# andrewkwolek/dynamic-visual-slam

Hardware: AMD Instinct MI355X
Metric: frames/sec ORB+match @1280x720x2000kp (higher is better)
Workload: dtype u8

## Files before the change

dynamic-visual-slam_amd/csrc/orb.hip:

```cpp
#include <math.h>
#include <stdlib.h>
#include <string.h>
#include <algorithm>
#include <new>
#include <vector>
#include "common.h"
#include "cv_round.h"
#include "device_mem.h"
#include "io_host.h"
#ifdef DVS_TEST_HOOKS
#include "../../include/dvslam_hip_test.h"
#endif
#include "orb_kernels.h"

namespace dvs {

void launch_cand_mask(const Geom* d_geom, const Cell* d_cells, const CandMask& mk, uint32_t* cand, int* cellCount, int nimg, int c0, int c1,
                      hipStream_t st);

static inline short sat_short(int v) { return (short)(v < -32768 ? -32768 : (v > 32767 ? 32767 : v)); }
static inline uint64_t align_up(uint64_t v, uint64_t a) { return (v + a - 1) / a * a; }

}

using namespace dvs;

// ... 110 lines not shown
  hipEvent_t after_fast_event = nullptr;
  hipEvent_t gate_event = nullptr;
  bool pf_joined = false;
  const u8* next_hint = nullptr;
  struct ChainGraph { const u8* img0; uint64_t step0, fstride0; int nimg; u8* pyr; hipGraph_t graph; hipGraphExec_t exec; };
  std::vector<ChainGraph> chain_graphs;
  int env_chain_graph = -1;
  int64_t chain_graph_launches = 0;
  bool pf_valid = false;
  const u8* pf_img = nullptr; uint64_t pf_step = 0, pf_fstride = 0; int pf_nimg = 0;
  int env_cascade = -1;
  int fast_byte_dma = 0;
  int env_blur_mfma = 0;
  int env_oct_threads = 0;
  int env_host_poll = 1;
  int env_desc_order = 1;
  PinnedBuf<int> h_seq;
  DeviceBuf<int> d_ticket;
  int export_seq = 0;
  bool async_oct = false, last_async = false;
  hipStream_t tail_stream = nullptr;
  CandMask mask{};
  int last_nimg = 0;
  ImgSrc last_src{};
  StageTimer timer;
};

namespace {

void drop_chain_graphs(dvs_orb* h) {
// ... 364 lines not shown
  DVS_TRY(W.d_geom.upload(std::vector<Geom>(1, G)));
  DVS_TRY(W.d_cells.upload(tb.cells));
  DVS_TRY(W.d_tiles.upload(tb.tiles));
  DVS_TRY(W.d_strips.upload(tb.strips));
  {
    std::vector<BlurCol> bcols; std::vector<uint4> btab;
    W.blur_mfma_ok = build_blur_mfma(G, bcols, btab, W.blur_avt);
    if (W.blur_mfma_ok) { DVS_TRY(W.d_blurcols.upload(bcols)); DVS_TRY(W.d_blurtab.upload(btab)); W.n_blurcols = (int)bcols.size(); }
  }
  DVS_TRY(W.d_rgroups.upload(tb.rgroups));
  DVS_TRY(W.d_pyrtiles.upload(tb.ptiles));
  if (G.pyrLds > 0) DVS_HIP(hipFuncSetAttribute((const void*)k_pyr_cascade<256>, hipFuncAttributeMaxDynamicSharedMemorySize, 2 * G.pyrLds));
  DVS_TRY(W.d_xofs.upload(tb.xofs)); DVS_TRY(W.d_alpha.upload(tb.alpha));
  DVS_TRY(W.d_yofs.upload(tb.yofs)); DVS_TRY(W.d_beta.upload(tb.beta));
  DVS_TRY(W.ready(W.pyr.cur()));
  DVS_TRY(W.ready(W.blur.cur()));
  DVS_TRY(W.ready(W.cand.cur()));
  DVS_TRY(W.d_pts.alloc(B * G.ptsPerFrame));
  DVS_TRY(W.d_nodeof.alloc(B * G.ptsPerFrame));
  DVS_TRY(W.d_celloff.alloc(B * G.totalCells));
  DVS_TRY(W.d_candtotal.alloc(B * G.nlevels));
  for (int k = 0; k < 3; k++) DVS_TRY(W.ready(W.lvl.at(k)));
  DVS_TRY(W.d_kpsorted.alloc(B * (size_t)G.kpBlock));
  DVS_TRY(W.d_kpsortidx.alloc(B * (size_t)G.kpBlock));
  {
    std::vector<uint32_t> ident(B * (size_t)G.kpBlock);
    for (size_t f = 0; f < B; f++)
      for (int l = 0; l < G.nlevels; l++) {
        const int end = l + 1 < G.nlevels ? G.lv[l + 1].kpOff : G.kpBlock;
        for (int sl = G.lv[l].kpOff; sl < end; sl++) ident[f * G.kpBlock + sl] = (uint32_t)(sl - G.lv[l].kpOff);
      }
// ... 203 lines not shown
  hipStream_t st = h->stream;
  const bool aligned0 = (((uintptr_t)src.img0) | src.step0 | src.fstride0) % 4 == 0;
  const uint32_t allLevels = G.nlevels >= 32 ? ~0u : ((1u << G.nlevels) - 1u);
  const bool sharded = (src.levelMask & allLevels) != allLevels || src.slotted;
  const bool prefetched = h->pf_valid && h->overlap && h->pf_img == src.img0 && h->pf_step == src.step0 &&
                          h->pf_fstride == src.fstride0 && h->pf_nimg == nimg;
  h->pf_valid = false;
  bool pend = h->out_pending;
  h->out_pending = false;
  if (pend && !(prefetched && may_defer)) {
    DVS_HIP(hipStreamWaitEvent(st, h->ev_outs.cur(), 0));
    pend = false;
  }
  const bool will_defer = h->overlap && may_defer && h->output_event && h->defer_outputs && !sharded;
  const bool async = h->async_oct && prefetched && will_defer && aligned0;
  if (async) {
    DVS_TRY(W.turn(W.cand));
    if (h->tail_stream) DVS_TRY(W.turn(W.blur));
  } else if (h->last_async) {
    DVS_HIP(hipStreamWaitEvent(st, W.cand.cur().done, 0));
  }
  h->last_async = async;
  h->async_run = async ? h->async_run + 1 : 0;

  if (prefetched) {
    W.pyr.take();
    if (!h->pf_joined) DVS_HIP(hipStreamWaitEvent(st, h->ev[kEvPrefetch + h->pf_idx], 0));
  }
  h->pf_joined = false;
  src.pyr = W.pyr.cur().pyr.get();
  int topLevel = 0;
  for (int l = 0; l < G.nlevels; l++) if ((src.levelMask >> l) & 1u) topLevel = l;
  const bool want_cascade = h->env_cascade >= 0 ? h->env_cascade == 1 : nimg <= 8;
// ... 11 lines not shown
      DVS_HIP(hipEventRecord(h->ev[kEvStart], st));
      DVS_HIP(hipStreamWaitEvent(pst, h->ev[kEvStart], 0));
    }
    h->timer.begin(DVS_STAGE_PYRAMID, pst);
    DVS_TRY(launch_pyramid_chain(h, src, nimg, W.pyr.cur().pyr.get(), pst, ov, sharded ? topLevel : -1));
    h->timer.end(pst);
  }
  if (next_img0 && h->overlap && G.nlevels >= 2) DVS_TRY(launch_prefetch(h, src, nimg, next_img0, pend));

  if (h->overlap) {
    if (h->guard_event && !will_defer) { DVS_HIP(hipStreamWaitEvent(h->aux_stream, h->guard_event, 0)); h->guard_event = nullptr; }
    if (h->pf_valid && !sharded && !(h->defer_outputs && h->output_event)) { DVS_HIP(hipStreamWaitEvent(h->aux_stream, h->ev[kEvPrefetch + h->pf_idx], 0)); h->pf_joined = true; }
  }

  const bool tail = async && h->tail_stream != nullptr;
  if (tail) {
    h->timer.begin(DVS_STAGE_BLUR, st);
    launch_blur(h, src, nimg, st, cascade);
    h->timer.end(st);
  }

  if (ov) {
    int tail = G.nlevels;
    while (tail > 2 && G.lv[tail - 1].nCells * 16 < G.totalCells) tail--;
    for (int l = 0; l <= tail && l < G.nlevels; l++) {
      const int lastl = l == tail ? G.nlevels - 1 : l;
      if (lastl > 0) DVS_HIP(hipStreamWaitEvent(st, h->ev_level[lastl], 0));
      h->timer.begin(DVS_STAGE_FAST, st, l == 0);
      launch_fast(h, src, nimg, st, G.lv[l].cellBase, G.lv[lastl].cellBase + G.lv[lastl].nCells);
      h->timer.end(st);
    }
// ... 5 lines not shown
    } else {
      launch_fast(h, src, nimg, st, 0, G.totalCells);
    }
    h->timer.end(st);
  }
  hipStream_t bst = h->overlap ? h->aux_stream : st;
  hipEvent_t ev_fastdone = h->after_fast_event ? h->after_fast_event : h->ev[kEvFork];
  if (h->after_fast_event || h->overlap) DVS_HIP(hipEventRecord(ev_fastdone, st));

  if (pend) {
    DVS_TRY(W.turn(W.lvl));
  }
  hipStream_t qs = async ? bst : st;
  if (async) DVS_HIP(hipStreamWaitEvent(bst, ev_fastdone, 0));
  const int blurRows = (G.blurStrips + kOctTMax / 64 - 1) / (kOctTMax / 64);
  const bool fuse_blur = h->single_stream && !async && !sharded && !(h->env_blur_mfma && W.blur_mfma_ok) &&
                         blur_stream_ok(h, src, cascade) && (long)nimg * (G.nlevels + blurRows) <= 256;
  h->timer.begin(DVS_STAGE_OCTREE, qs);
  if (fuse_blur) {
    if (h->guard_event) { DVS_HIP(hipStreamWaitEvent(qs, h->guard_event, 0)); h->guard_event = nullptr; }
    hipLaunchKernelGGL(k_octree_blur, dim3(nimg, G.nlevels + blurRows), dim3(kOctTMax), W.octree_smem, qs, W.d_geom.get(), W.cand.cur().cand.get(), W.cand.cur().cellcount.get(),
                       W.d_celloff.get(), W.d_pts.get(), W.d_nodeof.get(), W.d_candtotal.get(), W.lvl.cur().lvlkp.get(), W.lvl.cur().lvlcount.get(), W.octree_nmax, W.octree_ptscap, src.levelMask,
                       G.nlevels, W.d_strips.get(), G.blurStrips, src, W.blur.cur().blur.get());
  } else {
    launch_octree(h, nimg, qs, src.levelMask, async && G.nlevels * nimg > 256);
  }
  h->timer.end(qs);
  if (async) { DVS_HIP(hipEventRecord(W.cand.cur().done, qs)); W.cand.cur().done_valid = true; }

  if (async) {}
  else if (bst != st) DVS_HIP(hipStreamWaitEvent(bst, ev_fastdone, 0));
  else if (h->guard_event) DVS_HIP(hipStreamWaitEvent(st, h->guard_event, 0));
  hipEvent_t late_guard = bst != st ? h->guard_event : nullptr;
  h->guard_event = nullptr;
  if (!tail && !fuse_blur) {
    h->timer.begin(DVS_STAGE_BLUR, bst);
    launch_blur(h, src, nimg, bst, cascade);
    h->timer.end(bst);
  }

  hipStream_t dst = st;
  if (will_defer) {
    dst = tail ? h->tail_stream : bst;
    if (tail) {
      DVS_HIP(hipStreamWaitEvent(dst, W.cand.cur().done, 0));
    } else if (!async) {
      DVS_HIP(hipEventRecord(h->ev[kEvOct], st));
      DVS_HIP(hipStreamWaitEvent(bst, h->ev[kEvOct], 0));
    }
    if (late_guard) DVS_HIP(hipStreamWaitEvent(dst, late_guard, 0));
  } else if (bst != st) {
    DVS_HIP(hipEventRecord(h->ev[kEvBlur], bst));
    DVS_HIP(hipStreamWaitEvent(st, h->ev[kEvBlur], 0));
  }
  h->timer.begin(DVS_STAGE_DESCRIBE, dst);
  if (h->env_desc_order && nimg >= 16) {
    hipLaunchKernelGGL(k_kp_order, dim3(nimg, G.nlevels), dim3(256), 0, dst, W.d_geom.get(), W.lvl.cur().lvlkp.get(), W.lvl.cur().lvlcount.get(), W.d_kpsorted.get(), W.d_kpsortidx.get());
    hipLaunchKernelGGL(k_describe, dim3((G.kpBlock + 4 * kDescKP - 1) / (4 * kDescKP), nimg), dim3(256), 0, dst, W.d_geom.get(), src, W.blur.cur().blur.get(),
                       W.d_kpsorted.get(), W.d_kpsortidx.get(), W.lvl.cur().lvlcount.get(), d_kps, d_desc, d_nout, capacity);
  } else {
    hipLaunchKernelGGL(k_describe, dim3((G.kpBlock + 4 * kDescKP - 1) / (4 * kDescKP), nimg), dim3(256), 0, dst, W.d_geom.get(), src, W.blur.cur().blur.get(),
                       W.lvl.cur().lvlkp.get(), W.d_kpident.get(), W.lvl.cur().lvlcount.get(), d_kps, d_desc, d_nout, capacity);
  }
  h->timer.end(dst);
  if (will_defer) {
    h->ev_outs.advance();
    h->out_gen++;
    DVS_HIP(hipEventRecord(h->ev_outs.cur(), dst));
    DVS_HIP(hipEventRecord(h->output_event, dst));
    h->out_pending = true;
    h->gate_event = nullptr;
  } else {
    h->gate_event = (may_defer && h->output_event) ? h->output_event : h->ev[kEvEnd];
    DVS_HIP(hipEventRecord(h->gate_event, st));
  }
  DVS_HIP(hipGetLastError());
  h->last_nimg = nimg;
  h->last_src = src;
// ... 34 lines not shown
  if (on_stream) {
    h->stream = ext;
  } else {
    const hipError_t e = h->own_stream.create();
    if (e != hipSuccess) { delete h; set_error("hipStreamCreate: %s", hipGetErrorString(e)); return DVS_ERR_HIP; }
    h->stream = h->own_stream;
  }
  h->single_stream = single_stream;
  h->overlap = env_int("DVS_NO_OVERLAP", 0) == 0 && !single_stream;
  h->env_cascade = env_int("DVS_CASCADE", -1);
  h->env_chain_graph = env_int("DVS_CHAIN_GRAPH", -1);
  h->env_blur_mfma = env_int("DVS_BLUR_MFMA", 0);
  h->env_host_poll = env_int("DVS_HOST_POLL", 1);
  h->env_oct_threads = env_int("DVS_OCT_T", 0);
  h->env_desc_order = env_int("DVS_DESC_ORDER", 1);
  if (h->env_oct_threads != 0 && h->env_oct_threads != kOctT && h->env_oct_threads != kOctTMax) h->env_oct_threads = 0;
  h->fast_byte_dma = probe_byte_dma(device, h->stream) && env_int("DVS_FAST_BYTE_DMA", 1);
  bool ok = single_stream || (h->aux_stream.create(-1) == hipSuccess && h->pf_stream.create(1) == hipSuccess);
  for (Event& e : h->ev) ok = ok && e.create() == hipSuccess;
  for (Event& e : h->ev_outs.slot) ok = ok && e.create() == hipSuccess;
  for (int l = 1; l < params->nlevels; l++) ok = ok && h->ev_level[l].create() == hipSuccess;
  h->ev_outs.rewind(h->ring - 1);
  if (!ok) {
    dvs_orb_destroy(h);
    set_error("stream / event creation failed");
    return DVS_ERR_HIP;
  }
  build_ctor_tables(h);
  *out = h;
  return DVS_OK;
// ... 263 lines not shown
                                  dvs_keypoint* kps, uint8_t* desc, int32_t capacity, int32_t* n_out) {
  DVS_ARG(h && n_out);
  *n_out = 0;
  if (!gray || rows <= 0 || cols <= 0) { set_error("empty image"); return DVS_ERR_EMPTY; }
  const uint8_t* one[1] = {gray};
  const uint8_t* onem[1] = {mask};
  return dvs_orb_extract_batch_masked(h, one, 1, rows, cols, step, mask ? onem : nullptr, mask_step, kps, desc, capacity, n_out);
}

dvs_status dvs_orb_get_level(dvs_orb* h, int32_t frame, int32_t level, int32_t blurred, uint8_t* dst, int32_t cap_bytes) {
  DVS_ARG(h && dst && h->ws.d_geom.get() && frame >= 0 && frame < h->last_nimg && level >= 0 && level < h->ws.geom.nlevels);
  const LevelGeom& L = h->ws.geom.lv[level];
  if ((int64_t)L.w * L.h > cap_bytes) return DVS_ERR_CAPACITY;
  DVS_HIP(hipSetDevice(h->device));
  DVS_HIP(hipStreamSynchronize(h->stream));
  if (level == 0 && !blurred) {
    DVS_HIP(hipMemcpy2D(dst, L.w, h->last_src.img0 + (uint64_t)frame * h->last_src.fstride0, h->last_src.step0, L.w, L.h, hipMemcpyDeviceToHost));
  } else {
    const u8* base = (blurred ? h->ws.blur.cur().blur.get() : h->ws.pyr.cur().pyr.get()) + (uint64_t)frame * h->ws.geom.frameBytes + L.off;
    DVS_HIP(hipMemcpy2D(dst, L.w, base, L.pitch, L.w, L.h, hipMemcpyDeviceToHost));
  }
  return DVS_OK;
}

static dvs_status read_packed(dvs_orb* h, const uint32_t* dsrc, int n, int32_t* xys) {
  std::vector<uint32_t> tmp(n);
  if (n) DVS_HIP(hipMemcpy(tmp.data(), dsrc, (size_t)n * 4, hipMemcpyDeviceToHost));
  for (int i = 0; i < n; i++) { xys[3 * i] = pt_x(tmp[i]); xys[3 * i + 1] = pt_y(tmp[i]); xys[3 * i + 2] = pt_s(tmp[i]); }
  return DVS_OK;
}
// ... 6 lines not shown
  DVS_HIP(hipMemcpy(&cnt, h->ws.d_candtotal.get() + frame * h->ws.geom.nlevels + level, 4, hipMemcpyDeviceToHost));
  *n = cnt;
  if (cnt > cap) return DVS_ERR_CAPACITY;
  return read_packed(h, h->ws.d_pts.get() + (uint64_t)frame * h->ws.geom.ptsPerFrame + h->ws.geom.lv[level].ptsOff, cnt, xys);
}

DVS_HOOK dvs_status dvs_orb_get_level_keypoints(dvs_orb* h, int32_t frame, int32_t level, int32_t* xys, int32_t cap, int32_t* n) {
  DVS_ARG(h && xys && n && h->ws.d_geom.get() && frame >= 0 && frame < h->last_nimg && level >= 0 && level < h->ws.geom.nlevels);
  DVS_HIP(hipSetDevice(h->device));
  DVS_HIP(hipStreamSynchronize(h->stream));
  int cnt = 0;
  DVS_HIP(hipMemcpy(&cnt, h->ws.lvl.cur().lvlcount.get() + frame * h->ws.geom.nlevels + level, 4, hipMemcpyDeviceToHost));
  *n = cnt;
  if (cnt > cap) return DVS_ERR_CAPACITY;
  return read_packed(h, h->ws.lvl.cur().lvlkp.get() + (uint64_t)frame * h->ws.geom.kpBlock + h->ws.geom.lv[level].kpOff, cnt, xys);
}

DVS_HOOK dvs_status dvs_orb_enable_stage_timing(dvs_orb* h, int32_t on) {
  DVS_ARG(h);
  h->timer.resolve();
  h->timer.on = on != 0;
  return DVS_OK;
}

DVS_HOOK dvs_status dvs_orb_get_stage_times(dvs_orb* h, double* ms, int64_t* calls, int32_t reset) {
  DVS_ARG(h);
  DVS_HIP(hipSetDevice(h->device));
  DVS_HIP(hipStreamSynchronize(h->stream));
  h->timer.resolve();
  for (int i = 0; i < DVS_STAGE_COUNT; i++) { if (ms) ms[i] = h->timer.ms[i]; if (calls) calls[i] = h->timer.calls[i]; }
// ... 62 lines not shown
```

dynamic-visual-slam_amd/csrc/orb_kernels.h:

```cpp
#pragma once
#include <hip/hip_runtime.h>
#include "glibc_sincosf.h"
#include "lsort.h"
#include "orb_geom.h"
#include "orb_device_common.h"

namespace dvs {

typedef uint8_t u8;

struct ImgSrc {
  const u8* img0;
  uint64_t step0;
  uint64_t fstride0;
  u8* pyr;
  uint32_t levelMask;
  int32_t slotted;
};

__device__ __forceinline__ const u8* level_ptr(const Geom* g, const ImgSrc& s, int f, int l, int& pitch) {
  if (l == 0) { pitch = (int)s.step0; return s.img0 + (uint64_t)f * s.fstride0; }
  pitch = g->lv[l].pitch;
  return s.pyr + (uint64_t)f * g->frameBytes + g->lv[l].off;
}
// ... 1653 lines not shown
  uint32_t* outI = sortedIdx + (uint64_t)f * g->kpBlock + L.kpOff;
  for (int i = threadIdx.x; i < n; i += 256) {
    const uint32_t pk = in[i];
    key[i] = ((uint32_t)(pt_y(pk) >> 5) << 20) | ((uint32_t)(pt_x(pk) >> 7) << 12) | (uint32_t)i;
  }
  __syncthreads();
  for (int i = threadIdx.x; i < n; i += 256) {
    const uint32_t k = key[i];
    int rank = 0;
    for (int j = 0; j < n; j++) rank += key[j] < k ? 1 : 0;
    outK[rank] = in[i];
    outI[rank] = (uint32_t)i;
  }
}

__global__ __launch_bounds__(256) void k_describe(const Geom* __restrict__ g, ImgSrc src, const u8* __restrict__ blur,
                                                  const uint32_t* __restrict__ lvlKp, const uint32_t* __restrict__ lvlKpIdx, const int* __restrict__ lvlKpCount,
                                                  dvs_keypoint* __restrict__ outKp, u8* __restrict__ outDesc,
                                                  int* __restrict__ nOut, int capacity) {
  typedef uint4 __attribute__((aligned(1))) uint4u;
  __shared__ __attribute__((aligned(16))) u8 win[4][2][kWinRows * kWinPitch];
  DVS_CHAIN_PRIO();
  const int wg = xcd_contiguous_id();
  const int f = wg / (int)gridDim.x, bx = wg - f * (int)gridDim.x;
  const int lane = lane_id();
  const int wv = __builtin_amdgcn_readfirstlane(threadIdx.x >> 6);
  const int nl = g->nlevels;
  const int* cnt = lvlKpCount + f * nl;
  const int slot0 = (bx * 4 + wv) * kDescKP;
  if (bx == 0 && threadIdx.x == 0) {
    if (src.slotted) {
      for (int l = 0; l < nl; l++) nOut[f * nl + l] = cnt[l];
    } else {
      int total = 0;
      for (int l = 0; l < nl; l++) total += cnt[l];
      nOut[f] = min(total, capacity);
// ... 22 lines not shown
  const int pitchL = lvl == 0 ? (int)src.step0 : g->lv[lvl].pitch;
  const u8* blurL = blur + pyrOff;
  const int bpL = g->lv[lvl].pitch;
#define DVS_RL(v, i) __builtin_amdgcn_readlane((int)(v), (i))
#define DVS_RLP(p, i) reinterpret_cast<const u8*>(((uint64_t)(uint32_t)DVS_RL((uint32_t)((uint64_t)(p) >> 32), i) << 32) | (uint32_t)DVS_RL((uint32_t)(uint64_t)(p), i))
  const int prow = min(lane >> 1, 2 * kHalfPatch), half = lane & 1;
  const int v = prow - kHalfPatch;
  const int pcol = half ? 1 : -kHalfPatch;
  uint4 d[kDescKP];
#pragma unroll
  for (int i = 0; i < kDescKP; i++) {
    const u8* ib = DVS_RLP(imgL, i);
    const int pi = DVS_RL(pitchL, i), xi = DVS_RL(x, i), yi = DVS_RL(y, i);
    d[i] = *reinterpret_cast<const uint4u*>(ib + (uint32_t)(mul_i24(yi + v, pi) + xi + pcol));
  }
  const int e0 = lane, e1 = 64 + lane;
  const int wr0 = e0 / 3, wc0 = e0 - 3 * wr0, wr1 = min(e1 / 3, kWinRows - 1), wc1 = e1 - 3 * (e1 / 3);
  const bool w1ok = e1 < kWinRows * 3;
  static_assert(kDescKP == 8, "the window registers below are named per keypoint");
  uint4 wq0_0, wq0_1, wq0_2, wq0_3, wq0_4, wq0_5, wq0_6, wq0_7, wq1_0, wq1_1, wq1_2, wq1_3, wq1_4, wq1_5, wq1_6, wq1_7;
#define DVS_REQUEST_WINDOW(i)                                                                                  \
  {                                                                                                            \
    const u8* bb = DVS_RLP(blurL, i);                                                                          \
    const int bp = DVS_RL(bpL, i), xi = DVS_RL(x, i), yi = DVS_RL(y, i);                                       \
    const int xa = (xi - kWinR) & ~3;   \
    const u8* o = bb + (int64_t)(yi - kWinR) * bp + xa;                                                        \
    wq0_##i = *reinterpret_cast<const uint4*>(o + (uint32_t)(mul_i24(wr0, bp) + 16 * wc0));                    \
    wq1_##i = *reinterpret_cast<const uint4*>(o + (uint32_t)(mul_i24(wr1, bp) + 16 * wc1));                    \
  }
  DVS_REQUEST_WINDOW(0) DVS_REQUEST_WINDOW(1) DVS_REQUEST_WINDOW(2) DVS_REQUEST_WINDOW(3)
  float px0[4], py0[4], px1[4], py1[4];
#pragma unroll
  for (int r = 0; r < 4; r++) {
    const int pat = reinterpret_cast<const int*>(c_pattern)[64 * r + lane];
    px0[r] = (float)(int8_t)(pat & 0xff); py0[r] = (float)(int8_t)((pat >> 8) & 0xff);
    px1[r] = (float)(int8_t)((pat >> 16) & 0xff); py1[r] = (float)(int8_t)((pat >> 24) & 0xff);
  }
  const uint32_t* wt = g->icw[lane];
  const uint32_t w0 = wt[0], w1 = wt[1], w2 = wt[2], w3 = wt[3], w4 = wt[4], w5 = wt[5], w6 = wt[6], w7 = wt[7];
  int q[2 * kDescKP];
#pragma unroll
  for (int i = 0; i < kDescKP; i++) {
    uint32_t su = __builtin_amdgcn_udot4(d[i].x, w0, 0u, false);
    su = __builtin_amdgcn_udot4(d[i].y, w1, su, false);
    su = __builtin_amdgcn_udot4(d[i].z, w2, su, false);
    su = __builtin_amdgcn_udot4(d[i].w, w3, su, false);
    uint32_t sm = __builtin_amdgcn_udot4(d[i].x, w4, 0u, false);
    sm = __builtin_amdgcn_udot4(d[i].y, w5, sm, false);
    sm = __builtin_amdgcn_udot4(d[i].z, w6, sm, false);
    sm = __builtin_amdgcn_udot4(d[i].w, w7, sm, false);
    q[i] = (int)su - kHalfPatch * (int)sm;
    q[kDescKP + i] = v * (int)sm;
  }
  DVS_REQUEST_WINDOW(4) DVS_REQUEST_WINDOW(5) DVS_REQUEST_WINDOW(6) DVS_REQUEST_WINDOW(7)
#define DVS_BFLY(n, o)                                        \
  {                                                           \
    const bool hi = (lane & (o)) != 0;                        \
    _Pragma("unroll") for (int j = 0; j < (n); j++) {         \
      const int keep = hi ? q[(n) + j] : q[j];                \
      const int send = hi ? q[j] : q[(n) + j];                \
      q[j] = keep + __shfl_xor(send, (o));                    \
    }                                                         \
  }
  DVS_BFLY(8, 32) DVS_BFLY(4, 16) DVS_BFLY(2, 8) DVS_BFLY(1, 4)
#undef DVS_BFLY
  int tot = q[0];
  tot += __shfl_xor(tot, 2);
  tot += __shfl_xor(tot, 1);
  const int other = __shfl_xor(tot, 32);
// ... 28 lines not shown
      const float fr0 = rowv[0], fr1 = rowv[1], fc0 = colv[0], fc1 = colv[1];
      const int r0 = __builtin_bit_cast(int, fr0), r1 = __builtin_bit_cast(int, fr1);
      const int c0 = __builtin_bit_cast(int, fc0), c1 = __builtin_bit_cast(int, fc1);
      const int t0 = wl[mad_i24(r0, kWinPitch, c0) + bco];
      const int t1 = wl[mad_i24(r1, kWinPitch, c1) + bco];
      words[r] = __ballot(t0 < t1);
    }
    if ((vmask >> i) & 1u) {
      const int gii = DVS_RL(giL, i);
      if (lane < 4) {
        const unsigned long long w = lane == 0 ? words[0] : lane == 1 ? words[1] : lane == 2 ? words[2] : words[3];
        reinterpret_cast<unsigned long long*>(outDesc + ((uint64_t)f * capacity + gii) * 32)[lane] = w;
      }
    }
  };
  brief(0, wq0_0, wq1_0); brief(1, wq0_1, wq1_1); brief(2, wq0_2, wq1_2); brief(3, wq0_3, wq1_3);
  brief(4, wq0_4, wq1_4); brief(5, wq0_5, wq1_5); brief(6, wq0_6, wq1_6); brief(7, wq0_7, wq1_7);
  const float angle = __shfl(angleK, kCsLane * (lane & 7));
  if (lane < kDescKP && valid) {
    dvs_keypoint kp;
    kp.x = (float)x; kp.y = (float)y;
    if (level != 0) { kp.x = __fmul_rn(kp.x, L.scale); kp.y = __fmul_rn(kp.y, L.scale); }
    kp.size = L.kpSize;
    kp.angle = angle;
    kp.response = (float)pt_s(pk);
    kp.octave = level;
    kp.class_id = -1;
    outKp[(uint64_t)f * capacity + gi] = kp;
  }
#undef DVS_REQUEST_WINDOW
#undef DVS_RL
#undef DVS_RLP
// ... 56 lines not shown
```

dynamic-visual-slam_amd/csrc/util.hip:

```cpp
#include <stdlib.h>
#include <string.h>
#include "common.h"
#ifdef DVS_TEST_HOOKS
#include "../../include/dvslam_hip_test.h"
#include "block_ops.h"
#include "device_mem.h"
#endif

extern "C" char** environ;

namespace dvs {

static thread_local char g_err[1024] = "";

void set_error(const char* fmt, ...) {
  va_list ap;
  va_start(ap, fmt);
  vsnprintf(g_err, sizeof(g_err), fmt, ap);
  va_end(ap);
}

namespace {
struct EnvSwitch { const char* name; int allowed[4]; int nallowed; };
const EnvSwitch kSwitches[] = {
    {"DVS_NO_OVERLAP", {0, 1}, 2},
    {"DVS_CASCADE", {-1, 0, 1}, 3},
    {"DVS_CHAIN_GRAPH", {-1, 0, 1}, 3},
    {"DVS_BLUR_MFMA", {0, 1, 2}, 3},
    {"DVS_HOST_POLL", {0, 1}, 2},
    {"DVS_OCT_T", {0, 256, 512}, 3},
    {"DVS_DESC_ORDER", {0, 1}, 2},
    {"DVS_FAST_BYTE_DMA", {0, 1}, 2},
    {"DVS_MATCH_MFMA", {0, 1}, 2},
    {"DVS_MATCH_LDS", {0, 1}, 2},
    {"DVS_LM_POLL", {0, 1}, 2},
    {"DVS_LM_SPECULATE", {0, 1}, 2},
};
const EnvSwitch* find_switch(const char* name, size_t len) {
  for (const EnvSwitch& s : kSwitches)
    if (strlen(s.name) == len && strncmp(s.name, name, len) == 0) return &s;
  return nullptr;
}
}

dvs_status env_check() {
  for (char** e = environ; e && *e; e++) {
    if (strncmp(*e, "DVS_", 4) != 0) continue;
    const char* eq = strchr(*e, '=');
    if (!eq) continue;
    const EnvSwitch* s = find_switch(*e, (size_t)(eq - *e));
    if (!s) {
      set_error("unknown environment switch %.*s (the library reads: DVS_NO_OVERLAP DVS_CASCADE DVS_CHAIN_GRAPH DVS_BLUR_MFMA DVS_HOST_POLL DVS_OCT_T "
                "DVS_DESC_ORDER DVS_FAST_BYTE_DMA DVS_MATCH_MFMA DVS_MATCH_LDS DVS_LM_POLL DVS_LM_SPECULATE)", (int)(eq - *e), *e);
      return DVS_ERR_ARG;
    }
    char* end = nullptr;
    const long v = strtol(eq + 1, &end, 10);
    bool ok = end != eq + 1 && *end == 0;
    if (ok) { ok = false; for (int i = 0; i < s->nallowed; i++) ok = ok || s->allowed[i] == (int)v; }
    if (!ok) {
      char list[64] = ""; size_t o = 0;
      for (int i = 0; i < s->nallowed; i++) o += (size_t)snprintf(list + o, sizeof(list) - o, "%s%d", i ? ", " : "", s->allowed[i]);
      set_error("%s=%s: not a value of this switch (allowed: %s)", s->name, eq + 1, list);
      return DVS_ERR_ARG;
    }
  }
  return DVS_OK;
}
// ... 255 lines not shown
```

dynamic-visual-slam_amd/dvslam_amd/_lib.py:

```python
import ctypes as C
import os
import subprocess
import numpy as np

_PKG = os.path.dirname(os.path.dirname(os.path.abspath(__file__)))
SO_PATH = os.environ.get("DVSLAM_HIP_SO") or os.path.join(_PKG, "lib", "libdvslam_hip.so")

KP_DTYPE = np.dtype([("x", "<f4"), ("y", "<f4"), ("size", "<f4"), ("angle", "<f4"), ("response", "<f4"),
                     ("octave", "<i4"), ("class_id", "<i4")])

STATUS = {0: "DVS_OK", -1: "DVS_ERR_EMPTY", -2: "DVS_ERR_UNSUPPORTED", -3: "DVS_ERR_CAPACITY", -4: "DVS_ERR_HIP",
          -5: "DVS_ERR_NO_DEVICE", -6: "DVS_ERR_ARG"}


class DvsError(RuntimeError):
    def __init__(self, code, msg):
        super().__init__(f"{STATUS.get(code, code)}: {msg}")
        self.code = code


class OrbParams(C.Structure):
    _fields_ = [("nfeatures", C.c_int32), ("scale_factor", C.c_float), ("nlevels", C.c_int32), ("ini_th_fast", C.c_int32),
                ("min_th_fast", C.c_int32), ("gauss_kernel", C.c_int32 * 7), ("max_batch", C.c_int32)]

# ... 260 lines not shown
def _bind_hooks(L):
    vp, i32, sz, dbl = C.c_void_p, C.c_int32, C.c_size_t, C.c_double
    L.dvs_orb_use_own_stream.argtypes = [vp]
    L.dvs_orb_set_overlap.argtypes = [vp, i32]
    L.dvs_matcher_use_own_stream.argtypes = [vp]
    L.dvs_orb_hint_next_batch_device.argtypes = [vp, vp]
    L.dvs_orb_set_after_fast_event.argtypes = [vp, vp]
    L.dvs_orb_set_output_event.argtypes = [vp, vp]
    L.dvs_orb_set_defer_outputs.argtypes = [vp, i32]
    L.dvs_orb_set_reuse_guard_event.argtypes = [vp, vp]
    L.dvs_orb_set_async_quadtree.argtypes = [vp, i32]
    L.dvs_orb_set_tail_stream.argtypes = [vp, vp]
    L.dvs_orb_chain_graph_launches.argtypes = [vp]; L.dvs_orb_chain_graph_launches.restype = C.c_int64
    L.dvs_orb_get_candidates.argtypes = [vp, i32, i32, vp, i32, C.POINTER(i32)]
    L.dvs_orb_get_level_keypoints.argtypes = [vp, i32, i32, vp, i32, C.POINTER(i32)]
    L.dvs_orb_enable_stage_timing.argtypes = [vp, i32]
    L.dvs_orb_get_stage_times.argtypes = [vp, vp, vp, i32]
    L.dvs_orb_create_single_stream.argtypes = [C.POINTER(OrbParams), i32, C.POINTER(vp)]
    L.dvs_orb_create_on_stream.argtypes = [C.POINTER(OrbParams), i32, vp, C.POINTER(vp)]
    L.dvs_pipeline_extractor.argtypes = [vp]; L.dvs_pipeline_extractor.restype = vp
    L.dvs_pipeline_matcher.argtypes = [vp]; L.dvs_pipeline_matcher.restype = vp
    L.dvs_pipeline_match_stream.argtypes = [vp]; L.dvs_pipeline_match_stream.restype = vp


def lib():
    global _lib
    if _lib is not None:
        return _lib
    if not os.path.exists(SO_PATH):
        raise RuntimeError(f"{SO_PATH} not found: build it with `make -C {_PKG}` (hipcc --offload-arch=gfx950); "
# ... 147 lines not shown
```

dynamic-visual-slam_amd/dvslam_amd/orb.py:

```python
import ctypes as C
import numpy as np
from ._lib import lib, test_lib, check, ptr, OrbParams, KP_DTYPE, DvsError

STAGES = ("pyramid", "fast", "octree", "blur", "describe")


class ORBextractor:

    def __init__(self, nfeatures=1000, scaleFactor=1.2, nlevels=8, iniThFAST=20, minThFAST=7, device=0, max_batch=1,
                 gauss_kernel=None, hooks=False):
        self._L = test_lib() if hooks else lib()
        self.hooks = bool(hooks)
        p = OrbParams(nfeatures, scaleFactor, nlevels, iniThFAST, minThFAST, (C.c_int32 * 7)(*(gauss_kernel or [0] * 7)), max_batch)
        h = C.c_void_p()
        check(self._L.dvs_orb_create(C.byref(p), device, C.byref(h)))
        self._h = h
        self.nfeatures, self.nlevels, self.scaleFactor, self.device, self.max_batch = nfeatures, nlevels, scaleFactor, device, max_batch
        self.capacity = self._L.dvs_orb_max_keypoints(self._h)
        self._honour_mask = False

    @classmethod
    def from_handle(cls, handle, nfeatures, nlevels, scaleFactor, device, max_batch, L=None):
        o = cls.__new__(cls)
        o._L, o._h, o._owned = (L or lib()), C.c_void_p(handle), False
# ... 170 lines not shown

    def candidates(self, l, frame=0):
        cap = 1 << 20
        buf = np.zeros((cap, 3), np.int32)
        n = C.c_int32()
        check(self._L.dvs_orb_get_candidates(self._h, frame, l, ptr(buf), cap, C.byref(n)))
        return buf[:n.value].copy()

    def level_keypoints(self, l, frame=0):
        cap = self.nfeatures + 64
        buf = np.zeros((cap, 3), np.int32)
        n = C.c_int32()
        check(self._L.dvs_orb_get_level_keypoints(self._h, frame, l, ptr(buf), cap, C.byref(n)))
        return buf[:n.value].copy()

    def enable_stage_timing(self, on=True):
        check(self._L.dvs_orb_enable_stage_timing(self._h, int(on)))

    def stage_times(self, reset=True):
        ms = np.zeros(5, np.float64); calls = np.zeros(5, np.int64)
        check(self._L.dvs_orb_get_stage_times(self._h, ptr(ms), ptr(calls), int(reset)))
        return dict(zip(STAGES, ms.tolist())), dict(zip(STAGES, calls.tolist()))
```

Measured before the change: 149,100.

## Fuse Gaussian blur into describe kernel for large deferred batches

Adds an inline-blur variant of k_describe that blurs a small window around each keypoint in LDS using packed dot-product instructions, instead of relying on a separate full-image blur pass. For large deferred batches it skips the whole blur kernel and the write and read of the blurred pyramid. The blurred image is then produced lazily only when a debug accessor asks for it. The cost is redundant blur work where keypoint windows overlap, more register and LDS pressure in describe, and a slower border path.

```diff
diff --git a/dynamic-visual-slam_amd/csrc/orb.hip b/dynamic-visual-slam_amd/csrc/orb.hip
--- a/dynamic-visual-slam_amd/csrc/orb.hip
+++ b/dynamic-visual-slam_amd/csrc/orb.hip
@@ -10,6 +10,7 @@
 #include "io_host.h"
 #ifdef DVS_TEST_HOOKS
 #include "../../include/dvslam_hip_test.h"
+#include "../../include/dvslam_hip_test_describe.h"
 #endif
 #include "orb_kernels.h"
 
@@ -150,6 +151,8 @@
   int env_blur_mfma = 0;
   int env_oct_threads = 0;
   int env_host_poll = 1;
+  int env_desc_inline = -1;
+  bool blur_current = false;
   int env_desc_order = 1;
   PinnedBuf<int> h_seq;
   DeviceBuf<int> d_ticket;
@@ -544,7 +547,6 @@
   DVS_TRY(W.d_xofs.upload(tb.xofs)); DVS_TRY(W.d_alpha.upload(tb.alpha));
   DVS_TRY(W.d_yofs.upload(tb.yofs)); DVS_TRY(W.d_beta.upload(tb.beta));
   DVS_TRY(W.ready(W.pyr.cur()));
-  DVS_TRY(W.ready(W.blur.cur()));
   DVS_TRY(W.ready(W.cand.cur()));
   DVS_TRY(W.d_pts.alloc(B * G.ptsPerFrame));
   DVS_TRY(W.d_nodeof.alloc(B * G.ptsPerFrame));
@@ -778,9 +780,12 @@
   }
   const bool will_defer = h->overlap && may_defer && h->output_event && h->defer_outputs && !sharded;
   const bool async = h->async_oct && prefetched && will_defer && aligned0;
+  constexpr int kInlineBlurMinBatch = 64;
+  const bool inline_blur = h->env_desc_inline >= 0 ? h->env_desc_inline == 1 : (will_defer && nimg >= kInlineBlurMinBatch && !h->env_blur_mfma);
+  if (!inline_blur) DVS_TRY(W.ready(W.blur.cur()));
   if (async) {
     DVS_TRY(W.turn(W.cand));
-    if (h->tail_stream) DVS_TRY(W.turn(W.blur));
+    if (h->tail_stream && !inline_blur) DVS_TRY(W.turn(W.blur));
   } else if (h->last_async) {
     DVS_HIP(hipStreamWaitEvent(st, W.cand.cur().done, 0));
   }
@@ -822,7 +827,7 @@
   }
 
   const bool tail = async && h->tail_stream != nullptr;
-  if (tail) {
+  if (tail && !inline_blur) {
     h->timer.begin(DVS_STAGE_BLUR, st);
     launch_blur(h, src, nimg, st, cascade);
     h->timer.end(st);
@@ -858,7 +863,7 @@
   hipStream_t qs = async ? bst : st;
   if (async) DVS_HIP(hipStreamWaitEvent(bst, ev_fastdone, 0));
   const int blurRows = (G.blurStrips + kOctTMax / 64 - 1) / (kOctTMax / 64);
-  const bool fuse_blur = h->single_stream && !async && !sharded && !(h->env_blur_mfma && W.blur_mfma_ok) &&
+  const bool fuse_blur = !inline_blur && h->single_stream && !async && !sharded && !(h->env_blur_mfma && W.blur_mfma_ok) &&
                          blur_stream_ok(h, src, cascade) && (long)nimg * (G.nlevels + blurRows) <= 256;
   h->timer.begin(DVS_STAGE_OCTREE, qs);
   if (fuse_blur) {
@@ -877,7 +882,7 @@
   else if (h->guard_event) DVS_HIP(hipStreamWaitEvent(st, h->guard_event, 0));
   hipEvent_t late_guard = bst != st ? h->guard_event : nullptr;
   h->guard_event = nullptr;
-  if (!tail && !fuse_blur) {
+  if (!tail && !fuse_blur && !inline_blur) {
     h->timer.begin(DVS_STAGE_BLUR, bst);
     launch_blur(h, src, nimg, bst, cascade);
     h->timer.end(bst);
@@ -898,14 +903,17 @@
     DVS_HIP(hipStreamWaitEvent(st, h->ev[kEvBlur], 0));
   }
   h->timer.begin(DVS_STAGE_DESCRIBE, dst);
-  if (h->env_desc_order && nimg >= 16) {
+  const bool ordered = h->env_desc_order && nimg >= 16;
+  if (ordered)
     hipLaunchKernelGGL(k_kp_order, dim3(nimg, G.nlevels), dim3(256), 0, dst, W.d_geom.get(), W.lvl.cur().lvlkp.get(), W.lvl.cur().lvlcount.get(), W.d_kpsorted.get(), W.d_kpsortidx.get());
-    hipLaunchKernelGGL(k_describe, dim3((G.kpBlock + 4 * kDescKP - 1) / (4 * kDescKP), nimg), dim3(256), 0, dst, W.d_geom.get(), src, W.blur.cur().blur.get(),
-                       W.d_kpsorted.get(), W.d_kpsortidx.get(), W.lvl.cur().lvlcount.get(), d_kps, d_desc, d_nout, capacity);
-  } else {
-    hipLaunchKernelGGL(k_describe, dim3((G.kpBlock + 4 * kDescKP - 1) / (4 * kDescKP), nimg), dim3(256), 0, dst, W.d_geom.get(), src, W.blur.cur().blur.get(),
-                       W.lvl.cur().lvlkp.get(), W.d_kpident.get(), W.lvl.cur().lvlcount.get(), d_kps, d_desc, d_nout, capacity);
-  }
+  const uint32_t* kpv = ordered ? W.d_kpsorted.get() : W.lvl.cur().lvlkp.get();
+  const uint32_t* kpi = ordered ? W.d_kpsortidx.get() : W.d_kpident.get();
+  const dim3 dgrid((G.kpBlock + 4 * kDescKP - 1) / (4 * kDescKP), nimg);
+  if (inline_blur)
+    hipLaunchKernelGGL(k_describe<true>, dgrid, dim3(256), 0, dst, W.d_geom.get(), src, (const u8*)nullptr, kpv, kpi, W.lvl.cur().lvlcount.get(), d_kps, d_desc, d_nout, capacity);
+  else
+    hipLaunchKernelGGL(k_describe<false>, dgrid, dim3(256), 0, dst, W.d_geom.get(), src, (const u8*)W.blur.cur().blur.get(), kpv, kpi, W.lvl.cur().lvlcount.get(), d_kps, d_desc, d_nout, capacity);
+  h->blur_current = !inline_blur;
   h->timer.end(dst);
   if (will_defer) {
     h->ev_outs.advance();
@@ -970,6 +978,7 @@
   h->env_host_poll = env_int("DVS_HOST_POLL", 1);
   h->env_oct_threads = env_int("DVS_OCT_T", 0);
   h->env_desc_order = env_int("DVS_DESC_ORDER", 1);
+  h->env_desc_inline = env_int("DVS_DESC_INLINE_BLUR", -1);
   if (h->env_oct_threads != 0 && h->env_oct_threads != kOctT && h->env_oct_threads != kOctTMax) h->env_oct_threads = 0;
   h->fast_byte_dma = probe_byte_dma(device, h->stream) && env_int("DVS_FAST_BYTE_DMA", 1);
   bool ok = single_stream || (h->aux_stream.create(-1) == hipSuccess && h->pf_stream.create(1) == hipSuccess);
@@ -1263,6 +1272,12 @@
   if ((int64_t)L.w * L.h > cap_bytes) return DVS_ERR_CAPACITY;
   DVS_HIP(hipSetDevice(h->device));
   DVS_HIP(hipStreamSynchronize(h->stream));
+  if (blurred && !h->blur_current) {
+    DVS_TRY(h->ws.ready(h->ws.blur.cur()));
+    launch_blur(h, h->last_src, h->last_nimg, h->stream, false);
+    DVS_HIP(hipStreamSynchronize(h->stream));
+    h->blur_current = true;
+  }
   if (level == 0 && !blurred) {
     DVS_HIP(hipMemcpy2D(dst, L.w, h->last_src.img0 + (uint64_t)frame * h->last_src.fstride0, h->last_src.step0, L.w, L.h, hipMemcpyDeviceToHost));
   } else {
@@ -1299,6 +1314,51 @@
   *n = cnt;
   if (cnt > cap) return DVS_ERR_CAPACITY;
   return read_packed(h, h->ws.lvl.cur().lvlkp.get() + (uint64_t)frame * h->ws.geom.kpBlock + h->ws.geom.lv[level].kpOff, cnt, xys);
+}
+
+DVS_HOOK dvs_status dvs_orb_describe_level_keypoints(dvs_orb* h, int32_t frame, const int32_t* counts, const int32_t* xys, int32_t inline_blur,
+                                                     dvs_keypoint* kps, uint8_t* desc, int32_t cap, int32_t* n_out) {
+  DVS_ARG(h && counts && xys && kps && desc && n_out && h->ws.d_geom.get() && frame >= 0 && frame < h->last_nimg);
+  Workspace& W = h->ws;
+  const Geom& G = W.geom;
+  DVS_HIP(hipSetDevice(h->device));
+  DVS_HIP(hipStreamSynchronize(h->stream));
+  std::vector<uint32_t> lk((size_t)G.kpBlock, 0u);
+  std::vector<int> cnt((size_t)h->last_nimg * G.nlevels, 0);
+  int total = 0;
+  for (int l = 0; l < G.nlevels; l++) {
+    const LevelGeom& L = G.lv[l];
+    DVS_ARG(counts[l] >= 0 && counts[l] <= L.N + 4);
+    for (int i = 0; i < counts[l]; i++, xys += 3) {
+      DVS_ARG(xys[0] >= kEdge && xys[0] < L.w - kEdge && xys[1] >= kEdge && xys[1] < L.h - kEdge && xys[2] >= 0 && xys[2] < 256);
+      lk[(size_t)L.kpOff + i] = pack_pt(xys[0] - kMinBorder, xys[1] - kMinBorder, xys[2]);
+    }
+    cnt[(size_t)frame * G.nlevels + l] = counts[l];
+    total += counts[l];
+  }
+  DVS_ARG(total <= cap && total <= G.outCap);
+  DVS_HIP(hipMemcpy(W.lvl.cur().lvlkp.get() + (uint64_t)frame * G.kpBlock, lk.data(), lk.size() * 4, hipMemcpyHostToDevice));
+  DVS_HIP(hipMemcpy(W.lvl.cur().lvlcount.get(), cnt.data(), cnt.size() * sizeof(int), hipMemcpyHostToDevice));
+  if (!inline_blur && !h->blur_current) {
+    DVS_TRY(W.ready(W.blur.cur()));
+    launch_blur(h, h->last_src, h->last_nimg, h->stream, false);
+    h->blur_current = true;
+  }
+  ImgSrc src = h->last_src;
+  src.slotted = 0;
+  const dim3 dgrid((G.kpBlock + 4 * kDescKP - 1) / (4 * kDescKP), h->last_nimg);
+  if (inline_blur)
+    hipLaunchKernelGGL(k_describe<true>, dgrid, dim3(256), 0, h->stream, W.d_geom.get(), src, (const u8*)nullptr, (const uint32_t*)W.lvl.cur().lvlkp.get(),
+                       (const uint32_t*)W.d_kpident.get(), (const int*)W.lvl.cur().lvlcount.get(), W.d_kps.get(), W.d_desc.get(), W.d_nout.get(), G.outCap);
+  else
+    hipLaunchKernelGGL(k_describe<false>, dgrid, dim3(256), 0, h->stream, W.d_geom.get(), src, (const u8*)W.blur.cur().blur.get(), (const uint32_t*)W.lvl.cur().lvlkp.get(),
+                       (const uint32_t*)W.d_kpident.get(), (const int*)W.lvl.cur().lvlcount.get(), W.d_kps.get(), W.d_desc.get(), W.d_nout.get(), G.outCap);
+  DVS_HIP(hipGetLastError());
+  DVS_HIP(hipStreamSynchronize(h->stream));
+  *n_out = total;
+  DVS_HIP(hipMemcpy(kps, W.d_kps.get() + (uint64_t)frame * G.outCap, (size_t)total * sizeof(dvs_keypoint), hipMemcpyDeviceToHost));
+  DVS_HIP(hipMemcpy(desc, W.d_desc.get() + (uint64_t)frame * G.outCap * 32, (size_t)total * 32, hipMemcpyDeviceToHost));
+  return DVS_OK;
 }
 
 DVS_HOOK dvs_status dvs_orb_enable_stage_timing(dvs_orb* h, int32_t on) {
diff --git a/dynamic-visual-slam_amd/csrc/orb_kernels.h b/dynamic-visual-slam_amd/csrc/orb_kernels.h
--- a/dynamic-visual-slam_amd/csrc/orb_kernels.h
+++ b/dynamic-visual-slam_amd/csrc/orb_kernels.h
@@ -1691,12 +1691,20 @@
   }
 }
 
+constexpr int kIbR = kWinR + 3, kIbRows = 2 * kIbR + 1;
+constexpr int kIbGroups = 10, kIbItems = kIbRows * kIbGroups;
+constexpr int kIbIters = (kIbItems + 63) / 64;
+constexpr int kIbPitch = 8 * kIbGroups, kIbWave = kIbRows * kIbPitch;
+typedef uint32_t IbWords __attribute__((ext_vector_type(3)));
+
+template <bool kInlineBlur>
 __global__ __launch_bounds__(256) void k_describe(const Geom* __restrict__ g, ImgSrc src, const u8* __restrict__ blur,
                                                   const uint32_t* __restrict__ lvlKp, const uint32_t* __restrict__ lvlKpIdx, const int* __restrict__ lvlKpCount,
                                                   dvs_keypoint* __restrict__ outKp, u8* __restrict__ outDesc,
                                                   int* __restrict__ nOut, int capacity) {
   typedef uint4 __attribute__((aligned(1))) uint4u;
-  __shared__ __attribute__((aligned(16))) u8 win[4][2][kWinRows * kWinPitch];
+  __shared__ __attribute__((aligned(16))) u8 lds[kInlineBlur ? 4 * kIbWave : 4 * 2 * kWinRows * kWinPitch];
+  u8 (*win)[2][kWinRows * kWinPitch] = reinterpret_cast<u8 (*)[2][kWinRows * kWinPitch]>(lds);
   DVS_CHAIN_PRIO();
   const int wg = xcd_contiguous_id();
   const int f = wg / (int)gridDim.x, bx = wg - f * (int)gridDim.x;
@@ -1749,6 +1757,33 @@
     const int pi = DVS_RL(pitchL, i), xi = DVS_RL(x, i), yi = DVS_RL(y, i);
     d[i] = *reinterpret_cast<const uint4u*>(ib + (uint32_t)(mul_i24(yi + v, pi) + xi + pcol));
   }
+  int ibT[kIbIters], ibM4[kIbIters], ibLds[kIbIters];
+  uint32_t ibA[kIbIters][3], ibB[kIbIters][3];
+  const int hsOff = wv * kIbWave;
+  typedef const IbWords __attribute__((address_space(1), aligned(1))) * IbWordsG;
+  const int Wl = g->lv[lvl].w, Hl = g->lv[lvl].h;
+  const unsigned innerMask = (unsigned)(__ballot(x >= kIbR && x + kIbR + 5 < Wl && y >= kIbR && y + kIbR < Hl) & 0xffull);
+  const int winOff = mul_i24(y - kIbR, pitchL) + x - kIbR;
+  auto ib_request = [&](const int i, uint32_t (&q)[kIbIters][3]) __attribute__((always_inline)) {
+    if (!((innerMask >> i) & 1u)) return;
+    const u8* wb = DVS_RLP(imgL, i) + (uint32_t)DVS_RL(winOff, i);
+    const uint32_t pi = (uint32_t)DVS_RL(pitchL, i);
+#pragma unroll
+    for (int it = 0; it < kIbIters; it++) {
+      const IbWords w = *(IbWordsG)(uintptr_t)(wb + mad_u24_s((uint32_t)ibT[it], pi, (uint32_t)ibM4[it]));
+      q[it][0] = w.x; q[it][1] = w.y; q[it][2] = w.z;
+    }
+  };
+  if constexpr (kInlineBlur) {
+#pragma unroll
+    for (int it = 0; it < kIbIters; it++) {
+      const int e = min(it * 64 + lane, kIbItems - 1);
+      ibT[it] = (e * 205) >> 11;
+      ibM4[it] = 4 * (e - kIbGroups * ibT[it]);
+      ibLds[it] = hsOff + ibT[it] * kIbPitch + 2 * ibM4[it];
+    }
+    ib_request(0, ibA);
+  }
   const int e0 = lane, e1 = 64 + lane;
   const int wr0 = e0 / 3, wc0 = e0 - 3 * wr0, wr1 = min(e1 / 3, kWinRows - 1), wc1 = e1 - 3 * (e1 / 3);
   const bool w1ok = e1 < kWinRows * 3;
@@ -1763,7 +1798,7 @@
     wq0_##i = *reinterpret_cast<const uint4*>(o + (uint32_t)(mul_i24(wr0, bp) + 16 * wc0));                    \
     wq1_##i = *reinterpret_cast<const uint4*>(o + (uint32_t)(mul_i24(wr1, bp) + 16 * wc1));                    \
   }
-  DVS_REQUEST_WINDOW(0) DVS_REQUEST_WINDOW(1) DVS_REQUEST_WINDOW(2) DVS_REQUEST_WINDOW(3)
+  if constexpr (!kInlineBlur) { DVS_REQUEST_WINDOW(0) DVS_REQUEST_WINDOW(1) DVS_REQUEST_WINDOW(2) DVS_REQUEST_WINDOW(3) }
   float px0[4], py0[4], px1[4], py1[4];
 #pragma unroll
   for (int r = 0; r < 4; r++) {
@@ -1787,7 +1822,7 @@
     q[i] = (int)su - kHalfPatch * (int)sm;
     q[kDescKP + i] = v * (int)sm;
   }
-  DVS_REQUEST_WINDOW(4) DVS_REQUEST_WINDOW(5) DVS_REQUEST_WINDOW(6) DVS_REQUEST_WINDOW(7)
+  if constexpr (!kInlineBlur) { DVS_REQUEST_WINDOW(4) DVS_REQUEST_WINDOW(5) DVS_REQUEST_WINDOW(6) DVS_REQUEST_WINDOW(7) }
 #define DVS_BFLY(n, o)                                        \
   {                                                           \
     const bool hi = (lane & (o)) != 0;                        \
@@ -1846,8 +1881,98 @@
       }
     }
   };
-  brief(0, wq0_0, wq1_0); brief(1, wq0_1, wq1_1); brief(2, wq0_2, wq1_2); brief(3, wq0_3, wq1_3);
-  brief(4, wq0_4, wq1_4); brief(5, wq0_5, wq1_5); brief(6, wq0_6, wq1_6); brief(7, wq0_7, wq1_7);
+  if constexpr (!kInlineBlur) {
+    brief(0, wq0_0, wq1_0); brief(1, wq0_1, wq1_1); brief(2, wq0_2, wq1_2); brief(3, wq0_3, wq1_3);
+    brief(4, wq0_4, wq1_4); brief(5, wq0_5, wq1_5); brief(6, wq0_6, wq1_6); brief(7, wq0_7, wq1_7);
+  } else {
+    const uint32_t q0 = (uint32_t)g->gk[0], q1 = (uint32_t)g->gk[1], q2 = (uint32_t)g->gk[2], q3 = (uint32_t)g->gk[3], q4 = (uint32_t)g->gk[4],
+                   q5 = (uint32_t)g->gk[5], q6 = (uint32_t)g->gk[6];
+    const uint32_t wA0 = q0 | q1 << 8 | q2 << 16 | q3 << 24, wB0 = q4 | q5 << 8 | q6 << 16;
+    const uint32_t wA1 = q0 << 8 | q1 << 16 | q2 << 24, wB1 = q3 | q4 << 8 | q5 << 16 | q6 << 24;
+    const uint32_t wA2 = q0 << 16 | q1 << 24, wB2 = q2 | q3 << 8 | q4 << 16 | q5 << 24, wC2 = q6;
+    const uint32_t wA3 = q0 << 24, wB3 = q1 | q2 << 8 | q3 << 16 | q4 << 24, wC3 = q5 | q6 << 8;
+    typedef unsigned short us2v __attribute__((ext_vector_type(2)));
+    const us2v k01 = {(unsigned short)q0, (unsigned short)q1}, k23 = {(unsigned short)q2, (unsigned short)q3}, k45 = {(unsigned short)q4, (unsigned short)q5};
+    auto ib_item = [&](const uint32_t a, const uint32_t b, const uint32_t c, const int at) __attribute__((always_inline)) {
+      const uint32_t h0 = __builtin_amdgcn_udot4(b, wB0, __builtin_amdgcn_udot4(a, wA0, 0u, false), false);
+      const uint32_t h1 = __builtin_amdgcn_udot4(b, wB1, __builtin_amdgcn_udot4(a, wA1, 0u, false), false);
+      const uint32_t h2 = __builtin_amdgcn_udot4(c, wC2, __builtin_amdgcn_udot4(b, wB2, __builtin_amdgcn_udot4(a, wA2, 0u, false), false), false);
+      const uint32_t h3 = __builtin_amdgcn_udot4(c, wC3, __builtin_amdgcn_udot4(b, wB3, __builtin_amdgcn_udot4(a, wA3, 0u, false), false), false);
+      *reinterpret_cast<uint2*>(lds + at) = make_uint2(__builtin_amdgcn_perm(h1, h0, 0x05040100u), __builtin_amdgcn_perm(h3, h2, 0x05040100u));
+    };
+    auto ib_border = [&](const int i) __attribute__((always_inline)) {
+      const u8* ib = DVS_RLP(imgL, i);
+      const int pi = DVS_RL(pitchL, i), xi = DVS_RL(x, i), yi = DVS_RL(y, i), wi = DVS_RL(Wl, i), hi = DVS_RL(Hl, i);
+#pragma unroll 1
+      for (int it = 0; it < kIbIters; it++) {
+        const int e = min(it * 64 + lane, kIbItems - 1);
+        const int t = (e * 205) >> 11, m4 = 4 * (e - kIbGroups * t);
+        const int ry = min(max(reflect101(yi - kIbR + t, hi), 0), hi - 1);
+        const u8* row = ib + (uint32_t)(ry * pi);
+        uint32_t w[3] = {0u, 0u, 0u};
+#pragma unroll
+        for (int k = 0; k < 12; k++) {
+          const int cx = min(max(reflect101(xi - kIbR + m4 + k, wi), 0), wi - 1);
+          w[k >> 2] |= (uint32_t)row[cx] << (8 * (k & 3));
+        }
+        ib_item(w[0], w[1], w[2], hsOff + t * kIbPitch + 2 * m4);
+      }
+    };
+    const uint32_t k6s = __builtin_amdgcn_readfirstlane(q6);
+    auto ib_step = [&](const int i, uint32_t (&cur)[kIbIters][3], uint32_t (&nxt)[kIbIters][3]) __attribute__((always_inline)) {
+      const bool live = ((vmask >> i) & 1u) != 0;
+      if (live) {
+        if ((innerMask >> i) & 1u) {
+#pragma unroll
+          for (int it = 0; it < kIbIters; it++) ib_item(cur[it][0], cur[it][1], cur[it][2], ibLds[it]);
+        } else {
+          ib_border(i);
+        }
+      }
+      if (i + 1 < kDescKP) ib_request(i + 1, nxt);
+      if (!live) return;
+      wave_lds_fence();
+      const float a = __builtin_bit_cast(float, DVS_RL(__builtin_bit_cast(int, cosK), kCsLane * i));
+      const float b = __builtin_bit_cast(float, DVS_RL(__builtin_bit_cast(int, sinK), kCsLane * i));
+      const int kOff = hsOff + kWinR * kIbPitch + 2 * kWinR - 32 * kIbPitch - 2 * 32;
+      auto blurred = [&](const int ri, const int ci) __attribute__((always_inline)) -> uint32_t {
+        const uint16_t* p = reinterpret_cast<const uint16_t*>(lds + mad_i24(ri, kIbPitch, mad_i24(ci, 2, kOff)));
+        constexpr int P = kIbPitch / 2;
+        const us2v r01 = {p[0], p[P]}, r23 = {p[2 * P], p[3 * P]}, r45 = {p[4 * P], p[5 * P]};
+        uint32_t acc = mad_u24_s((uint32_t)p[6 * P], k6s, 32768u);
+        acc = __builtin_amdgcn_udot2(r01, k01, acc, false);
+        acc = __builtin_amdgcn_udot2(r23, k23, acc, false);
+        acc = __builtin_amdgcn_udot2(r45, k45, acc, false);
+        return acc >> 16;
+      };
+      unsigned long long words[4];
+      typedef float f32x2 __attribute__((ext_vector_type(2)));
+      const f32x2 a2 = {a, a}, b2 = {b, b};
+#pragma unroll
+      for (int r = 0; r < 4; r++) {
+        constexpr float kRound = 8388640.0f;
+        const f32x2 kR2 = {kRound, kRound};
+        const f32x2 pxv = {px0[r], px1[r]}, pyv = {py0[r], py1[r]};
+        const f32x2 rowv = (pxv * b2 + pyv * a2) + kR2;
+        const f32x2 colv = (pxv * a2 - pyv * b2) + kR2;
+        const float fr0 = rowv[0], fr1 = rowv[1], fc0 = colv[0], fc1 = colv[1];
+        const uint32_t t0 = blurred(__builtin_bit_cast(int, fr0), __builtin_bit_cast(int, fc0));
+        const uint32_t t1 = blurred(__builtin_bit_cast(int, fr1), __builtin_bit_cast(int, fc1));
+        words[r] = __ballot(t0 < t1);
+      }
+      const int gii = DVS_RL(giL, i);
+      if (lane < 4) {
+        const unsigned long long w = lane == 0 ? words[0] : lane == 1 ? words[1] : lane == 2 ? words[2] : words[3];
+        reinterpret_cast<unsigned long long*>(outDesc + ((uint64_t)f * capacity + gii) * 32)[lane] = w;
+      }
+      wave_lds_fence();
+    };
+#pragma unroll 1
+    for (int i = 0; i < kDescKP; i += 2) {
+      ib_step(i, ibA, ibB);
+      ib_step(i + 1, ibB, ibA);
+    }
+  }
   const float angle = __shfl(angleK, kCsLane * (lane & 7));
   if (lane < kDescKP && valid) {
     dvs_keypoint kp;
diff --git a/dynamic-visual-slam_amd/csrc/util.hip b/dynamic-visual-slam_amd/csrc/util.hip
--- a/dynamic-visual-slam_amd/csrc/util.hip
+++ b/dynamic-visual-slam_amd/csrc/util.hip
@@ -30,6 +30,7 @@
     {"DVS_HOST_POLL", {0, 1}, 2},
     {"DVS_OCT_T", {0, 256, 512}, 3},
     {"DVS_DESC_ORDER", {0, 1}, 2},
+    {"DVS_DESC_INLINE_BLUR", {-1, 0, 1}, 3},
     {"DVS_FAST_BYTE_DMA", {0, 1}, 2},
     {"DVS_MATCH_MFMA", {0, 1}, 2},
     {"DVS_MATCH_LDS", {0, 1}, 2},
@@ -51,7 +52,7 @@
     const EnvSwitch* s = find_switch(*e, (size_t)(eq - *e));
     if (!s) {
       set_error("unknown environment switch %.*s (the library reads: DVS_NO_OVERLAP DVS_CASCADE DVS_CHAIN_GRAPH DVS_BLUR_MFMA DVS_HOST_POLL DVS_OCT_T "
-                "DVS_DESC_ORDER DVS_FAST_BYTE_DMA DVS_MATCH_MFMA DVS_MATCH_LDS DVS_LM_POLL DVS_LM_SPECULATE)", (int)(eq - *e), *e);
+                "DVS_DESC_ORDER DVS_DESC_INLINE_BLUR DVS_FAST_BYTE_DMA DVS_MATCH_MFMA DVS_MATCH_LDS DVS_LM_POLL DVS_LM_SPECULATE)", (int)(eq - *e), *e);
       return DVS_ERR_ARG;
     }
     char* end = nullptr;
diff --git a/dynamic-visual-slam_amd/dvslam_amd/_lib.py b/dynamic-visual-slam_amd/dvslam_amd/_lib.py
--- a/dynamic-visual-slam_amd/dvslam_amd/_lib.py
+++ b/dynamic-visual-slam_amd/dvslam_amd/_lib.py
@@ -298,6 +298,7 @@
     L.dvs_orb_chain_graph_launches.argtypes = [vp]; L.dvs_orb_chain_graph_launches.restype = C.c_int64
     L.dvs_orb_get_candidates.argtypes = [vp, i32, i32, vp, i32, C.POINTER(i32)]
     L.dvs_orb_get_level_keypoints.argtypes = [vp, i32, i32, vp, i32, C.POINTER(i32)]
+    L.dvs_orb_describe_level_keypoints.argtypes = [vp, i32, vp, vp, i32, vp, vp, i32, C.POINTER(i32)]
     L.dvs_orb_enable_stage_timing.argtypes = [vp, i32]
     L.dvs_orb_get_stage_times.argtypes = [vp, vp, vp, i32]
     L.dvs_orb_create_single_stream.argtypes = [C.POINTER(OrbParams), i32, C.POINTER(vp)]
diff --git a/dynamic-visual-slam_amd/dvslam_amd/orb.py b/dynamic-visual-slam_amd/dvslam_amd/orb.py
--- a/dynamic-visual-slam_amd/dvslam_amd/orb.py
+++ b/dynamic-visual-slam_amd/dvslam_amd/orb.py
@@ -208,6 +208,16 @@
         check(self._L.dvs_orb_get_level_keypoints(self._h, frame, l, ptr(buf), cap, C.byref(n)))
         return buf[:n.value].copy()
 
+    def describe_level_keypoints(self, per_level, inline_blur, frame=0):
+        counts = np.array([len(p) for p in per_level], np.int32)
+        xys = np.ascontiguousarray(np.concatenate([np.asarray(p, np.int32).reshape(-1, 3) for p in per_level]), np.int32)
+        kps = np.zeros(self.capacity, KP_DTYPE)
+        desc = np.zeros((self.capacity, 32), np.uint8)
+        n = C.c_int32()
+        check(self._L.dvs_orb_describe_level_keypoints(self._h, frame, ptr(counts), ptr(xys), int(bool(inline_blur)), ptr(kps), ptr(desc),
+                                                       self.capacity, C.byref(n)))
+        return n.value, kps[:n.value].copy(), desc[:n.value].copy()
+
     def enable_stage_timing(self, on=True):
         check(self._L.dvs_orb_enable_stage_timing(self._h, int(on)))
 
diff --git a/include/dvslam_hip_test_describe.h b/include/dvslam_hip_test_describe.h
--- /dev/null
+++ b/include/dvslam_hip_test_describe.h
@@ -0,0 +1,14 @@
+#ifndef DVSLAM_HIP_TEST_DESCRIBE_H
+#define DVSLAM_HIP_TEST_DESCRIBE_H
+#include "dvslam_hip.h"
+#ifdef __cplusplus
+extern "C" {
+#endif
+
+dvs_status dvs_orb_describe_level_keypoints(dvs_orb* h, int32_t frame, const int32_t* counts, const int32_t* xys, int32_t inline_blur,
+                                            dvs_keypoint* kps, uint8_t* desc, int32_t cap, int32_t* n_out);
+
+#ifdef __cplusplus
+}
+#endif
+#endif
```

Result: slower. 146,900 (-1.5%).
